# lijx10/USIP

Hardware: AMD Instinct MI355X
Metric: point-clouds/sec detector fwd+bwd (higher is better)
Workload: dtype f32 results; matrix-bound products emulated from 2 fp16 planes per operand (22-bit operands, 3 plane products, exact ...; 1 GPU; KITTI detector N=16384 M=512 K=64 batch=8 pairs/GPU (BASELINE configs[2]); detector=RPN_Detector_Ball, clouds_per_gpu=16, surface_normal_len=4, node_knn_k_1=16, ball_radius=2, ball_k=64, cloud=slab, matmul=f32x2, step=fwd+losses+bwd+adam, launch=HIP graph replay (ONE graph per step: forward, backward, Adam), parallelism=dp1

## Files before the change

include/usip_hip.h:

```cpp
#ifndef USIP_HIP_H
#define USIP_HIP_H

#include <stdint.h>

#ifdef __cplusplus
extern "C" {
#endif

#define USIP_OK      0
#define USIP_EINVAL (-1)
#define USIP_ABI 6

const char* usip_version(void);

enum { USIP_TUNE_INDEX_MAX_CH = 0, USIP_TUNE_INDEX_MAX_UNROLL, USIP_TUNE_X3_WGRAD_TILE, USIP_TUNE_X3_GEMM_TILE,
       USIP_TUNE_GEMM_SPLIT3, USIP_TUNE_INDEX_MAX_THREADS, USIP_TUNE_X2_DIRECT, USIP_TUNE_R5_FORMS, USIP_TUNE_COUNT };
int usip_set_tuning(const char* name, int value);
int usip_tuning_value(int knob);

int usip_launch_log(int on);
const char* usip_launch_log_entry(int i, unsigned* workgroups);

int usip_index_max_f32(const float* data, const int32_t* index, int32_t* max_idx,
                       int B, int C, int N, int K, void* stream);
// ... 137 lines not shown

int usip_mlp_gemm_x2d_red_tiles(int M, int K, int P, int nb, int red_group);
int usip_mlp_gemm_x2h_red_f32(const void* planes, const float* X, const float* X2, const float* coef, int pro,
                              const float* pool_dp, const int32_t* pool_arg, int pool_group, float* Y,
                              const float* red_y, const float* red_coef, float* red_out, float* red_gsum,
                              int red_group, int M, int K, int P, int nb, void* stream);
int usip_mlp_gemm_x2h_fork_supported(int M, int K, int P, int nb, int fork_group);
int usip_mlp_gemm_x2h_fork_f32(const void* planes, const float* X, const float* X2, const float* coef, float* Y, int y_rows,
                               const float* fork_dp, const int32_t* fork_arg, int fork_group, int M, int K, int P, int nb,
                               void* stream);
int usip_mlp_gemm_x2r_tiles(int P, int nb);
int usip_mlp_gemm_x2r_f32(const void* planes, const float* X, const float* X2, const float* coef, int pro,
                          const float* bias, const float* rowbias, int rb_group, const float* pool_dp,
                          const int32_t* pool_arg, int pool_group, float* Y, int y_rows, float* stats, int M, int K,
                          int P, int nb, void* stream);

int usip_multi_transpose_f32(const float* src, float* dst, const int32_t* table, int ntensors, int total_tiles,
                             void* stream);

int usip_bn_finalize_f32(const float* stats, int tiles, int C, long long count,
                         const float* gamma, const float* beta, float eps, float momentum,
                         float* running_mean, float* running_var, float* mean, float* invstd,
                         float* coef, void* stream);

int usip_bn_apply_f32(const float* Y, const float* coef, float* Z, int relu,
                      int nb, int C, int P, void* stream);

int usip_bn_backward_reduce_f32(const float* dZ, const float* Y, const float* coef_fwd,
                                const float* mean, const float* invstd, const float* gamma, int relu,
                                float* partial, float* dgamma, float* dbeta, float* coef4,
// ... 52 lines not shown
                        float* workspace, float* dW, int ldw, int coloff,
                        int M, int N, int P, int nb, void* stream);
int usip_mlp_wgrad_x2h_f32(const float* G, const float* G2, const float* coef, int pro, const float* X,
                        const float* xcoef, const float* pool_dp, const int32_t* pool_arg, int pool_group,
                        float* workspace, float* dW, int ldw, int coloff,
                        int M, int N, int P, int nb, void* stream);
int usip_mlp_wgrad_f32x3_used(int M, int N, int P, int nb);

int usip_group_gather_f32(const float* x, const int32_t* idx, const float* sub, float* out,
                          int B, int C, int N, int M, int K, int nsub, int Ctot, int coff, void* stream);
int usip_group_gather_backward_f32(const float* dout, const int32_t* idx, float* dx,
                                   int B, int C, int N, int M, int K, int Ctot, int coff, void* stream);
int usip_group_max_f32(const float* z, float* pooled, int32_t* arg, long long rows, int K, void* stream);
int usip_group_max_act_f32(const float* y, const float* coef, int relu, float* pooled, int32_t* arg, float* yarg,
                           int B, int C, int M, int K, void* stream);
int usip_group_max_backward_f32(const float* dpooled, const int32_t* arg, float* dz,
                                long long rows, int K, void* stream);
int usip_group_max_backward_add_f32(const float* dpooled, const int32_t* arg, float* dz,
                                    long long rows, int K, void* stream);

int usip_group_max_wide_f32(const float* y, const float* coef, int relu, float* pooled, int32_t* arg, float* yarg,
                            int B, int C, int M, int K, void* stream);
int usip_bn_backward_reduce_wide_f32(const float* dZ, const float* Y, const float* coef_fwd,
                                     const float* mean, const float* invstd, const float* gamma, int relu,
                                     float* partial, float* dgamma, float* dbeta, float* coef4,
                                     float* gsum, int group, int nb, int C, int P, int want_bound, void* stream);

int usip_knn_f32(const float* query, const float* database, int32_t* idx,
                 int B, int M, int N, int K, void* stream);

// ... 367 lines not shown
```

usip_amd/csrc/group.hip:

```cpp
#include "common.h"
#include "pool_order.h"

namespace {

__global__ __launch_bounds__(256) void group_gather_kernel(
    const float* __restrict__ x, const int32_t* __restrict__ idx, const float* __restrict__ sub,
    float* __restrict__ out, int C, int N, int M, int K, int nsub, int Ctot, int coff)
{
    const int b = blockIdx.y;
    const int P = M * K;
    const int p = blockIdx.x * 256 + threadIdx.x;
    if (p >= P) return;
    const int n = idx[(long long)b * P + p];
    const int m = p / K;
    const float* xb = x + (long long)b * C * N;
    float* ob = out + ((long long)b * Ctot + coff) * P;
    for (int c = 0; c < C; ++c) {
        float v = xb[(long long)c * N + n];
        if (c < nsub) v -= sub[((long long)b * nsub + c) * M + m];
        ob[(long long)c * P + p] = v;
    }
}

__global__ __launch_bounds__(256) void group_gather_bwd_kernel(
// ... 45 lines not shown
{
    return __builtin_bit_cast(float, __builtin_amdgcn_update_dpp(0, __builtin_bit_cast(int, v), CTRL, 0xF, 0xF, false));
}
template <int CTRL>
__device__ __forceinline__ int dpp_i(int v) { return __builtin_amdgcn_update_dpp(0, v, CTRL, 0xF, 0xF, false); }

template <int L, int CTRL>
__device__ __forceinline__ void argmax_step(float& best, int& bk, float& braw)
{
    const float ov = dpp_f<CTRL>(best);
    const int ok = dpp_i<CTRL>(bk);
    const float orw = dpp_f<CTRL>(braw);
    if (ov > best || (ov == best && ok < bk)) { best = ov; bk = ok; braw = orw; }
}

template <int L, bool NANS>
__global__ __launch_bounds__(256) void group_max4_kernel(
    const float* __restrict__ z, float* __restrict__ pooled, int32_t* __restrict__ arg, long long rows,
    const float* __restrict__ coef, int relu, int C, int M, float* __restrict__ zarg, int nbatch)
{
    constexpr int RPB = 256 / L, RPT = 4;
    const int sub = threadIdx.x % L;
    const bool small = rows < (1LL << 31);
    const long long first = (long long)blockIdx.x * nbatch;
    auto row_of = [&](long long batch, int j) { return batch * RPB * RPT + threadIdx.x / L + (long long)j * RPB; };
    float4 v[RPT], nv[RPT];
#pragma unroll
    for (int j = 0; j < RPT; ++j) v[j] = usip_load_stream4(z + (min(row_of(first, j), rows - 1) * L + sub) * 4);
    for (int bi = 0; bi < nbatch; ++bi) {
        const long long batch = first + bi;
        if (bi + 1 < nbatch) {
#pragma unroll
            for (int j = 0; j < RPT; ++j) nv[j] = usip_load_stream4(z + (min(row_of(batch + 1, j), rows - 1) * L + sub) * 4);
        }
#pragma unroll
        for (int j = 0; j < RPT; ++j) {
            const long long row = row_of(batch, j);
            float4 w = v[j];
            if (coef) {
                const int ch = small ? (int)(((unsigned)min(row, rows - 1) / (unsigned)M) % (unsigned)C)
                                     : (int)((min(row, rows - 1) / M) % C);
                const float s0 = coef[ch], s1 = coef[C + ch];
                w.x = __builtin_fmaf(w.x, s0, s1); w.y = __builtin_fmaf(w.y, s0, s1);
                w.z = __builtin_fmaf(w.z, s0, s1); w.w = __builtin_fmaf(w.w, s0, s1);
                if (relu) { w.x = fmaxf(w.x, 0.f); w.y = fmaxf(w.y, 0.f); w.z = fmaxf(w.z, 0.f); w.w = fmaxf(w.w, 0.f); }
            }
            float best = w.x, braw = v[j].x;
            int bk = sub * 4;
            if (pool_gt<NANS>(w.y, best)) { best = w.y; bk = sub * 4 + 1; braw = v[j].y; }
            if (pool_gt<NANS>(w.z, best)) { best = w.z; bk = sub * 4 + 2; braw = v[j].z; }
            if (pool_gt<NANS>(w.w, best)) { best = w.w; bk = sub * 4 + 3; braw = v[j].w; }
            if constexpr (NANS) pool_hide_nan(best, bk);
            if constexpr (L == 4 || L == 16) {
                argmax_step<L, 0xB1>(best, bk, braw);
                argmax_step<L, 0x4E>(best, bk, braw);
                if constexpr (L == 16) {
                    argmax_step<L, 0x141>(best, bk, braw);
                    argmax_step<L, 0x140>(best, bk, braw);
                }
            } else {
#pragma unroll
                for (int off = L / 2; off > 0; off >>= 1) {
                    const float ov = __shfl_xor(best, off);
                    const int ok = __shfl_xor(bk, off);
                    const float orw = __shfl_xor(braw, off);
                    if (ov > best || (ov == best && ok < bk)) { best = ov; bk = ok; braw = orw; }
                }
            }
            if (sub == 0 && row < rows) {
                if constexpr (NANS) {
                    if (bk < 0) { bk += POOL_NAN; best = coef ? __builtin_nanf("") : braw; }
                }
                pooled[row] = best;
                arg[row] = bk;
                if (zarg) zarg[row] = braw;
            }
        }
#pragma unroll
        for (int j = 0; j < RPT; ++j) v[j] = nv[j];
    }
}

static int group_max4_batches(long long batches)
{
    if (!(usip_tuning_value(USIP_TUNE_R5_FORMS) & 8)) return 1;
    int nb = 1;
    while (nb < 8 && batches / (nb * 2) >= 2048) nb *= 2;
    return nb;
}

__global__ __launch_bounds__(256) void group_max_bwd4_kernel(
    const float* __restrict__ dpooled, const int32_t* __restrict__ arg, float* __restrict__ dz,
    long long total4, int K4)
{
    const long long i = (long long)blockIdx.x * 256 + threadIdx.x;
    if (i >= total4) return;
    const long long row = i / K4;
    const int k = (int)(i - row * K4) * 4;
    const int a = arg[row] - k;
    const float g = dpooled[row];
    *reinterpret_cast<float4*>(dz + i * 4) =
        make_float4(a == 0 ? g : 0.f, a == 1 ? g : 0.f, a == 2 ? g : 0.f, a == 3 ? g : 0.f);
}
// ... 135 lines not shown
        const long long blocks = (batches + nbatch - 1) / nbatch;                                \
        if (blocks > 0x7fffffffLL) return USIP_EINVAL;                                           \
        if (relu)                                                                                \
            USIP_LAUNCH((group_max4_kernel<L_, false>), dim3((unsigned)blocks), dim3(256), 0, st, y, pooled, arg, rows, \
                        coef, relu, C, M, yarg, nbatch);                                        \
        else                                                                                     \
            USIP_LAUNCH((group_max4_kernel<L_, true>), dim3((unsigned)blocks), dim3(256), 0, st, y, pooled, arg, rows, \
                        coef, relu, C, M, yarg, nbatch);                                        \
    }
    USIP_GM4(1) USIP_GM4(2) USIP_GM4(4) USIP_GM4(8) USIP_GM4(16) USIP_GM4(32) USIP_GM4(64)
#undef USIP_GM4
    USIP_LAUNCH_CHECK();
    return USIP_OK;
}

extern "C" int usip_group_max_f32(const float* z, float* pooled, int32_t* arg, long long rows, int K,
                                  void* stream)
{
    if (rows < 0 || K < 1) return USIP_EINVAL;
    if (rows == 0) return USIP_OK;
    if (!z || !pooled || !arg) return USIP_EINVAL;
    hipStream_t st = (hipStream_t)stream;
    const int L4 = K / 4;
    if (K % 4 == 0 && (L4 & (L4 - 1)) == 0 && L4 <= 64 && (reinterpret_cast<uintptr_t>(z) & 15u) == 0) {
#define USIP_GM4(L_)                                                                             \
        if (L4 == L_) {                                                                          \
            const long long batches = (rows + 4 * (256 / L_) - 1) / (4 * (256 / L_));            \
            const int nbatch = group_max4_batches(batches);                                      \
            const long long blocks = (batches + nbatch - 1) / nbatch;                            \
            if (blocks > 0x7fffffffLL) return USIP_EINVAL;                                       \
// ... 59 lines not shown
```

usip_amd/csrc/shared_mlp_x3.hip:

```cpp
#include "mlp_common.h"
#include "split_common.h"
#include <type_traits>

using namespace usip_mlp;

namespace {

constexpr int X2H_PARTS = 32;

__device__ __forceinline__ float* x2h_trailer(const usip_split3_desc& d)
{
    const int bm = d.tile_rows, ksteps = (d.K + XBK - 1) / XBK;
    return reinterpret_cast<float*>(reinterpret_cast<unsigned char*>(d.planes) +
                                    (long long)((d.M + bm - 1) / bm) * ksteps * 2 * bm * 32);
}

__device__ __forceinline__ void absmax_part(const usip_split3_desc& d, int part)
{
    __shared__ float red[4];
    const long long total = (long long)d.M * d.K, per = (total + X2H_PARTS - 1) / X2H_PARTS;
    const long long i0 = part * per, i1 = i0 + per < total ? i0 + per : total;
    float mx = 0.f;
    for (long long i = i0 + threadIdx.x; i < i1; i += 256) {
        const int k = (int)(i / d.M), m = (int)(i % d.M);
// ... 744 lines not shown
#undef USIP_X2L_PRODUCT
#undef USIP_X2L_READ_FRAGS
    {
        const float out_scale = 1.0f / (gscale * xscale);
#pragma unroll
        for (int i = 0; i < TM; ++i)
#pragma unroll
            for (int j = 0; j < TN; ++j)
#pragma unroll
                for (int r = 0; r < 16; ++r) acc[i][j][r] *= out_scale;
    }
    wgrad_store_partial<TM, TN>(a, acc, slice, m0, n0, wm, wn, lane);
}


template <int PRO, int EPI, bool RB = false>
__global__ __launch_bounds__(256) __attribute__((amdgpu_waves_per_eu(2, 2))) void gemm_x2r_kernel(const GemmArgs a, const uint4* __restrict__ planes)
{
    constexpr bool POOL = (PRO == PRO_BN_BWD_POOL);
    constexpr bool TWO = (PRO == PRO_BN_BWD) || POOL;
    constexpr int NCOEF = TWO ? 4 : 2;
    constexpr int BN = 64, SLAB = 64, PLB = BN * SLAB * 2;
    __shared__ __attribute__((aligned(16))) unsigned char Bs[2][2][PLB];
    __shared__ float cf[NCOEF][128];
    __shared__ float redm[4];
    __shared__ float rbs[RB ? 2 : 1][RB ? 128 : 1][2];

    const int tid = threadIdx.x, lane = tid & 63;
    const int wave = __builtin_amdgcn_readfirstlane(tid >> 6);
    const int c = lane & 31, kh = lane >> 5;
    const int nk = (a.K + XBK - 1) / XBK;
    const int nslab = (a.K + SLAB - 1) / SLAB;
// ... 24 lines not shown
    bf16x8 fa[8][2];
    {
        const int row = wave * 32 + c;
        const int chunk = row * 2 + ((kh ^ (row >> 3)) & 1);
#pragma unroll
        for (int s8 = 0; s8 < 8; ++s8)
#pragma unroll
            for (int pl = 0; pl < 2; ++pl) {
                uint4 v = make_uint4(0u, 0u, 0u, 0u);
                if (s8 < nk) v = planes[(long long)(s8 * 2 + pl) * 256 + chunk];
                fa[s8][pl] = __builtin_bit_cast(bf16x8, v);
            }
    }
    __shared__ float bsh[128];
    if (tid < 128) bsh[tid] = (a.bias && tid < a.M) ? a.bias[tid] : 0.f;
    float s1[EPI == EPI_STATS ? 16 : 1], s2[EPI == EPI_STATS ? 16 : 1];
    if (EPI == EPI_STATS) {
#pragma unroll
        for (int r = 0; r < 16; ++r) { s1[r] = 0.f; s2[r] = 0.f; }
    }

    const int xp = tid & 63;
    const int xkg = wave;
    const int pgrp = POOL ? a.P / a.pool_group : 0;
    const unsigned cloud_bytes = (unsigned)a.K * (unsigned)a.P * 4u, pool_bytes = (unsigned)a.K * (unsigned)pgrp * 4u;

    struct Raw { float x[16]; float y[TWO ? 16 : 1]; int arg[POOL ? 16 : 1]; int xkin; float rb; };
    const int ngrp = RB ? a.P / a.rb_group : 0;
    auto load_slab = [&](int tile, int sl, Raw& r) {
        const int b = tile / tpc, p0 = (tile - b * tpc) * BN;
// ... 95 lines not shown
                        acc[j] = __builtin_amdgcn_mfma_f32_32x32x16_f16(__builtin_bit_cast(f16x8, w0), __builtin_bit_cast(f16x8, fb[1][j]), acc[j], 0, 0, 0);
                        acc[j] = __builtin_amdgcn_mfma_f32_32x32x16_f16(__builtin_bit_cast(f16x8, w1), __builtin_bit_cast(f16x8, fb[0][j]), acc[j], 0, 0, 0);
                        acc[j] = __builtin_amdgcn_mfma_f32_32x32x16_f16(__builtin_bit_cast(f16x8, w0), __builtin_bit_cast(f16x8, fb[0][j]), acc[j], 0, 0, 0);
                    }
                }
            }
        }
        if (q + 1 < nsteps) {
            store_slab(cur ^ 1, slab_of(q + 1), nxt, ((q + 1) / nslab) & 1);
            if (q + 1 + DIST < nsteps) load_slab(tile_of(q + 1 + DIST), slab_of(q + 1 + DIST), nxt);
        }
        if (sl == nslab - 1) {
            const int tile = tile_of(q);
            const int b = tile / tpc, pt = tile - b * tpc, p0 = pt * BN;
            float* yb = a.Y + (long long)b * a.y_rows * a.P;
#pragma unroll
            for (int j = 0; j < 2; ++j) {
                const int pp = p0 + j * 32 + c;
                const bool pok = pp < a.P;
#pragma unroll
                for (int r = 0; r < 16; ++r) {
                    const int ch = wave * 32 + 8 * (r >> 2) + 4 * kh + (r & 3);
                    float v = __builtin_fmaf(acc[j][r], out_scale, bsh[ch]);
                    if (RB) v += rbs[RB ? (q / nslab) & 1 : 0][RB ? ch : 0][j];
                    if (pok && ch < a.M) {
                        st_out<RB ? ST_X2R : ST_X2R_PLAIN>(yb + (long long)ch * a.P + pp, v);
                        if (EPI == EPI_STATS) { s1[EPI == EPI_STATS ? r : 0] += v; s2[EPI == EPI_STATS ? r : 0] = __builtin_fmaf(v, v, s2[EPI == EPI_STATS ? r : 0]); }
                    }
                }
            }
#pragma unroll
            for (int j = 0; j < 2; ++j)
#pragma unroll
                for (int r = 0; r < 16; ++r) acc[j][r] = 0.f;
        }
        asm volatile("s_waitcnt lgkmcnt(0)" ::: "memory");
        __builtin_amdgcn_s_barrier();
        cur ^= 1;
    };
    for (int q = 0; q < nsteps; q += 2) {
        step(q, DIST == 2 ? rB : rA);
        if (q + 1 < nsteps) step(q + 1, rA);
    }
    if (EPI == EPI_STATS) {
#pragma unroll
        for (int r = 0; r < 16; ++r) {
            float u = usip_row16_sum(s1[EPI == EPI_STATS ? r : 0]), v = usip_row16_sum(s2[EPI == EPI_STATS ? r : 0]);
            u += __shfl_xor(u, 16);
            v += __shfl_xor(v, 16);
            const int ch = wave * 32 + 8 * (r >> 2) + 4 * kh + (r & 3);
            if (c == 0 && ch < a.M) {
                a.stats[(long long)ch * G + blockIdx.x] = u;
                a.stats[(long long)G * a.M + (long long)ch * G + blockIdx.x] = v;
            }
        }
    }
}

}

extern "C" int usip_mlp_x3p_tile_rows(int M, int P, int nb)
{
    const int t = usip_tuning_value(USIP_TUNE_X3_GEMM_TILE);
    if (M <= 128 || t == 1) return 128;
    const long long wide = (long long)((M + 255) / 256) * nb * ((P + 127) / 128);
    return wide >= 256 ? 256 : 128;
}


extern "C" long long usip_mlp_split3_bytes(int M, int K)
{
// ... 215 lines not shown
    if (pro == PRO_AFFINE_RELU && rowbias) {
        if (stats) USIP_LAUNCH((gemm_x2r_kernel<PRO_AFFINE_RELU, EPI_STATS, true>), dim3(grid), dim3(256), 0, st, a, pl);
        else USIP_LAUNCH((gemm_x2r_kernel<PRO_AFFINE_RELU, EPI_NONE, true>), dim3(grid), dim3(256), 0, st, a, pl);
    } else if (pro == PRO_AFFINE_RELU) {
        if (stats) USIP_LAUNCH((gemm_x2r_kernel<PRO_AFFINE_RELU, EPI_STATS>), dim3(grid), dim3(256), 0, st, a, pl);
        else USIP_LAUNCH((gemm_x2r_kernel<PRO_AFFINE_RELU, EPI_NONE>), dim3(grid), dim3(256), 0, st, a, pl);
    } else if (pro == PRO_BN_BWD) {
        USIP_LAUNCH((gemm_x2r_kernel<PRO_BN_BWD, EPI_NONE>), dim3(grid), dim3(256), 0, st, a, pl);
    } else {
        USIP_LAUNCH((gemm_x2r_kernel<PRO_BN_BWD_POOL, EPI_NONE>), dim3(grid), dim3(256), 0, st, a, pl);
    }
    USIP_LAUNCH_CHECK();
    return USIP_OK;
}

namespace usip_mlp {

void wgrad_x3_plan(int M, int N, int P, int nb, int* seglen, int* segs, int* tiles)
{
    *tiles = ((M + 255) / 256) * ((N + 255) / 256);
    long long want = (usip_tuning_value(USIP_TUNE_X3_WGRAD_TILE) == 2 ? 512 : 256) / (*tiles);
    if (want < 1) want = 1;
    long long per_cloud = (want + nb - 1) / nb;
    if (per_cloud < 1) per_cloud = 1;
    long long sl = (P + per_cloud - 1) / per_cloud;
    sl = ((sl + 31) / 32) * 32;
    long long floor_sl = 512;
    if (usip_tuning_value(USIP_TUNE_X3_WGRAD_TILE) != 4)
        while (floor_sl > 128 && (long long)(*tiles) * nb * ((P + floor_sl - 1) / floor_sl) < 192) floor_sl /= 2;
    if (sl < floor_sl) sl = floor_sl;
// ... 36 lines not shown
```

usip_amd/functional.py:

```python
from typing import Optional, Tuple

import torch
import torch.nn.functional as F

from . import ops, prof


GRAD_SINK = False
DEFER_BN_COUNTERS = False


FUSED_NARROW_BWD = True
FUSED_NARROW_RED = True
import os as _os
if _os.environ.get("USIP_NARROW_BWD") is not None:
    FUSED_NARROW_BWD = _os.environ["USIP_NARROW_BWD"] not in ("0", "off")
if _os.environ.get("USIP_NARROW_RED") is not None:
    FUSED_NARROW_RED = _os.environ["USIP_NARROW_RED"] not in ("0", "off")


SEGMENT_BACKWARD = _os.environ.get("USIP_SEGMENT_BWD", "1") not in ("0", "off")


WT_CACHE = None
# ... 502 lines not shown
                dw = ops.mlp_wgrad(dz, x, pro=2, G2=y, coef4=coef4, xcoef=xcoef,
                                   out=sink[0].view(w2.shape) if sink else None)
        db = torch.zeros_like(gamma) if (ctx.needs_input_grad[3] and not sink) else None
        if sink:
            dw = db = dgamma = dbeta = None
        return (dx, None, dw, db, dgamma, dbeta) + tail


class _SharedMLPLayerMax(torch.autograd.Function):

    @staticmethod
    def forward(ctx, x, xcoef, dims, w2, bias, gamma, beta, running_mean, running_var, momentum, eps, sink):
        B, Cin, M, K = dims
        x3 = x.contiguous().view(B, Cin, M * K)
        Cout = w2.shape[0]
        y, stats = ops.mlp_gemm(_kmajor(w2), x3, bias, want_stats=True,
                                pro=0 if xcoef is None else 1, coef=xcoef)
        mean, invstd, coef = ops.bn_finalize(stats, B * M * K, gamma, beta, eps, momentum, running_mean, running_var)
        y = _relu_hook(y, coef)
        pooled, arg, yarg = _pooled_act(y.view(B, Cout, M, K), coef, True, want_yarg=True)
        ctx.save_for_backward(x3, xcoef, w2, y, coef, mean, invstd, gamma, arg, yarg)
        ctx.dims, ctx.sink, ctx.x_shape = (B, Cin, Cout, M, K), sink, tuple(x.shape)
        return pooled

    @staticmethod
    def backward(ctx, dpooled):
        x3, xcoef, w2, y, coef, mean, invstd, gamma, arg, yarg = ctx.saved_tensors
        B, Cin, Cout, M, K = ctx.dims
        sink = ctx.sink
        dpooled = dpooled.contiguous()
        dgamma, dbeta, coef4 = ops.bn_pool_backward_reduce(dpooled, arg, y.view(B, Cout, M, K), coef, mean, invstd,
                                                           gamma, True, dgamma_out=sink[2] if sink else None,
                                                           dbeta_out=sink[3] if sink else None, yarg=yarg)
        pool = (dpooled, arg, K)
        dx = dw = None
# ... 536 lines not shown
```

usip_amd/ops.py:

```python
import ctypes
import functools
import math
import os
import types
from typing import Callable, NamedTuple, Optional

import torch

from . import _lib, prof


def _stream(t: torch.Tensor):
    return ctypes.c_void_p(torch.cuda.current_stream(t.device).cuda_stream)


def _need(t: torch.Tensor, name: str, dtype):
    if not isinstance(t, torch.Tensor):
        raise RuntimeError("%s must be a torch.Tensor" % name)
    if not t.is_cuda:
        raise RuntimeError("%s must be a CUDA tensor/variable" % name)
    if not t.is_contiguous():
        raise RuntimeError("%s must be contiguous" % name)
    if t.dtype != dtype:
        raise RuntimeError("%s must be %s (got %s)" % (name, dtype, t.dtype))
# ... 489 lines not shown
        dt = np.dtype(_lib.STRUCTS["usip_split3_desc"])
        table = np.array(rows, dtype=dt) if rows else np.zeros(0, dtype=dt)
        dev = next(iter(self.entries.values()))[1].device if rows else None
        self.table = torch.from_numpy(table.view(np.uint8).copy()).to(dev) if rows else None

    def refresh(self):
        if self.table is not None:
            with torch.cuda.device(self.table.device), prof.kernel("weight_split3", 0.0):
                _lib.check(_lib.lib().usip_mlp_split3_multi_f32(_ptr(self.table), len(self.entries), self.blocks,
                                                                _stream(self.table)), "usip_mlp_split3_multi_f32")
        return dict(self.entries)


NARROW_FWD = _os.environ.get("USIP_NARROW_FWD", "1") not in ("0", "off")
POOL_GRAD_FOLD = _os.environ.get("USIP_POOL_GRAD_FOLD", "1") not in ("0", "off")


def mlp_gemm(At: torch.Tensor, X: torch.Tensor, bias=None, want_stats: bool = False, pro: int = 0,
             X2=None, coef=None, tag: str = "fwd", rowbias=None, rb_group: int = 1,
             M: Optional[int] = None, a_offset: int = 0, pool=None, a_trans: bool = False, out=None,
             out_row_offset: int = 0, red=None, red_group: int = 0, fork=None):
    _need(At, "At", torch.float32)
    if a_trans:
        M_rows, lda = At.shape
        M = M_rows if M is None else int(M)
        K = X2.shape[1] if X is None else X.shape[1]
    else:
        K, lda = At.shape
        M = lda if M is None else int(M)
    pool_dp = pool_arg = None
    pool_group = 0
    if pool is not None:
        pool_dp, pool_arg, pool_group = pool
        X = X2
    _need(X, "X", torch.float32)
    nb, Kx, P = X.shape
# ... 47 lines not shown
    red_tiles = 0
    if (red is not None and plain_dgrad and out is None
            and red[1] is not None and red[1].shape[0] >= 4 and tuple(red[0].shape) == (nb, M, P)
            and red[0].is_contiguous() and red[0].data_ptr() % 16 == 0):
        red_tiles = int(lib.usip_mlp_gemm_x2d_red_tiles(M, K, P, nb, int(red_group)))
    fork_fold = False
    if fork is not None and plain_dgrad and pro == 2 and red is None and not want_stats and POOL_GRAD_FOLD:
        f_dp, f_arg, f_group = fork
        _need(f_dp, "fork dpooled", torch.float32)
        _need(f_arg, "fork arg", torch.int32)
        fork_fold = bool(f_group > 0 and P % f_group == 0 and tuple(f_dp.shape) == (nb, M, P // f_group)
                         and f_arg.shape == f_dp.shape and f_dp.data_ptr() % 16 == 0 and f_arg.data_ptr() % 16 == 0
                         and X.data_ptr() % 16 == 0 and X2.data_ptr() % 16 == 0 and y_ptr.value % 16 == 0
                         and lib.usip_mlp_gemm_x2h_fork_supported(M, K, P, nb, int(f_group)))
    third = None
    x_ptr = None if pool is not None else _ptr(X)
    epi = (_opt(coef), int(pro), _opt(bias), _opt(rowbias), int(rb_group))
    pooled = (_opt(pool_dp), _opt(pool_arg), int(pool_group))
    shape = (M, K, P, nb, _stream(X))
    if nf_blocks:
        fn, args = "usip_mlp_narrow_forward_f32", (a_ptr, lda, x_ptr) + epi + (y_ptr, int(y_rows), _opt(stats))
    elif red_tiles:
        flat = torch.empty(2 * red_tiles * M + red_tiles * (M // 256), dtype=torch.float32, device=X.device)
        third = RedSums(flat, M, blocks=red_tiles)
        third.gsum = torch.empty((2, nb, M, P // red_group), dtype=torch.float32, device=X.device) if red_group else None
        fn, args = "usip_mlp_gemm_x2h_red_f32", (_ptr(planes), x_ptr, _opt(X2), _opt(coef), int(pro)) + pooled + (
            y_ptr, _ptr(red[0]), _ptr(red[1]), _ptr(flat), _opt(third.gsum), int(red_group))
    elif fork_fold:
        third = True
        fn, args = "usip_mlp_gemm_x2h_fork_f32", (_ptr(planes), _ptr(X), _ptr(X2), _ptr(coef), y_ptr, int(y_rows),
                                                  _ptr(f_dp), _ptr(f_arg), int(f_group))
    else:
        fn = (("usip_mlp_gemm_x2r_f32" if x2r else "usip_mlp_gemm_x2h_f32" if x2h else "usip_mlp_gemm_x3p_f32") if x3p else
              {"bf16": "usip_mlp_gemm_bf16", "f32x3": "usip_mlp_gemm_f32x3", "f32x2": "usip_mlp_gemm_f32x3"}.get(
                  _matmul_mode, "usip_mlp_gemm_f32"))
        args = ((_ptr(planes),) if x3p else (a_ptr, -lda if a_trans else lda)) + (x_ptr, _opt(X2)) + epi + pooled + (
            y_ptr, int(y_rows), _opt(stats))
    with torch.cuda.device(X.device), prof.kernel("shared_mlp_gemm_%s %dx%d" % (tag, M, K),
                                                  4.0 * nb * P * (K * (2 if pro == 2 else 1) + M),
                                                  2.0 * M * K * nb * P, keyed=True, moved=moved):
        _lib.check(getattr(lib, fn)(*args, *shape), fn)
    return (Y, stats, third) if red is not None else ((Y, stats, bool(third)) if fork is not None else (Y, stats))


def bn_finalize(stats, count, gamma, beta, eps, momentum, running_mean, running_var):
    _, C, tiles = stats.shape
    dev = stats.device
    mean = torch.empty(C, dtype=torch.float32, device=dev)
    invstd = torch.empty(C, dtype=torch.float32, device=dev)
    coef = torch.empty((4, C), dtype=torch.float32, device=dev)
    with torch.cuda.device(dev), prof.kernel("bn_finalize", 4.0 * 2 * tiles * C):
        _lib.check(_lib.lib().usip_bn_finalize_f32(_ptr(stats), tiles, C, int(count), _opt(gamma), _opt(beta),
                                                   float(eps), float(momentum), _opt(running_mean),
                                                   _opt(running_var), _ptr(mean), _ptr(invstd), _ptr(coef),
                                                   _stream(stats)), "usip_bn_finalize_f32")
    declare_samples(coef, int(count))
# ... 398 lines not shown
    return pooled, arg


def group_max_act(y4, coef, relu: bool, want_yarg: bool = False):
    _need(y4, "y", torch.float32)
    B, C, M, K = y4.shape
    pooled = torch.empty((B, C, M), dtype=torch.float32, device=y4.device)
    arg = torch.empty((B, C, M), dtype=torch.int32, device=y4.device)
    yarg = torch.empty((B, C, M), dtype=torch.float32, device=y4.device) if want_yarg else None
    with torch.cuda.device(y4.device), prof.kernel("group_max", 4.0 * B * C * M * (K + 2)):
        _lib.check(_lib.lib().usip_group_max_act_f32(_ptr(y4), _ptr(coef), int(bool(relu)), _ptr(pooled), _ptr(arg),
                                                     _opt(yarg), B, C, M, K, _stream(y4)), "usip_group_max_act_f32")
    return (pooled, arg, yarg) if want_yarg else (pooled, arg)


WIDE_GROUPS = os.environ.get("USIP_WIDE_GROUPS", "1") not in ("0", "off")


def wide_group_supported(K: int) -> bool:
    return bool(WIDE_GROUPS) and 256 < K <= 1024 and K % 32 == 0


def group_max_wide(y4, coef=None, relu: bool = False, want_yarg: bool = False):
    _need(y4, "y", torch.float32)
    B, C, M, K = y4.shape
    pooled = torch.empty((B, C, M), dtype=torch.float32, device=y4.device)
    arg = torch.empty((B, C, M), dtype=torch.int32, device=y4.device)
    yarg = torch.empty((B, C, M), dtype=torch.float32, device=y4.device) if want_yarg else None
    with torch.cuda.device(y4.device), prof.kernel("group_max_wide", 4.0 * B * C * M * (K + 2)):
        _lib.check(_lib.lib().usip_group_max_wide_f32(_ptr(y4), _opt(coef), int(bool(relu)), _ptr(pooled), _ptr(arg),
# ... 1706 lines not shown
```

Measured before the change: 4109 point-clouds/s.

## Fuse max-pool candidate scan into GEMM epilogue with cheap resolve kernel

The x2r GEMM epilogue now scans each 64-wide K group per output channel and records the top pre-activation value, the runner-up, the first element and the argmax, using the sign of gamma as the order key. A small resolve kernel then applies the BN affine and ReLU to those records to produce pooled, arg and yarg. It falls back to a full row rescan only on ties, non-finite values or sign mismatches. This is meant to avoid re-reading the whole Y tensor in a separate group-max pass, at the cost of extra LDS traffic and registers in the GEMM epilogue and a small candidate buffer.

After: 4136 point-clouds/s, median of 6. Within noise of the previous version (+0.7%).

```diff
diff --git a/include/usip_hip.h b/include/usip_hip.h
--- a/include/usip_hip.h
+++ b/include/usip_hip.h
@@ -175,6 +175,9 @@
                           const float* bias, const float* rowbias, int rb_group, const float* pool_dp,
                           const int32_t* pool_arg, int pool_group, float* Y, int y_rows, float* stats, int M, int K,
                           int P, int nb, void* stream);
+int usip_mlp_gemm_x2r_cand_f32(const void* planes, const float* X, const float* coef, const float* bias,
+                               const float* gamma, float* Y, int y_rows, float* stats, void* cand, int M, int K, int P,
+                               int nb, void* stream);
 
 int usip_multi_transpose_f32(const float* src, float* dst, const int32_t* table, int ntensors, int total_tiles,
                              void* stream);
@@ -257,6 +260,9 @@
 int usip_group_max_f32(const float* z, float* pooled, int32_t* arg, long long rows, int K, void* stream);
 int usip_group_max_act_f32(const float* y, const float* coef, int relu, float* pooled, int32_t* arg, float* yarg,
                            int B, int C, int M, int K, void* stream);
+int usip_pool_resolve_f32(const void* cand, const float* y, const float* coef, const float* gamma, int relu,
+                          float* pooled, int32_t* arg, float* yarg, int B, int C, int M, void* nfallback,
+                          void* stream);
 int usip_group_max_backward_f32(const float* dpooled, const int32_t* arg, float* dz,
                                 long long rows, int K, void* stream);
 int usip_group_max_backward_add_f32(const float* dpooled, const int32_t* arg, float* dz,
diff --git a/usip_amd/csrc/group.hip b/usip_amd/csrc/group.hip
--- a/usip_amd/csrc/group.hip
+++ b/usip_amd/csrc/group.hip
@@ -1,5 +1,6 @@
 #include "common.h"
 #include "pool_order.h"
+#include "pool_cand.h"
 
 namespace {
 
@@ -83,6 +84,48 @@
     if (ov > best || (ov == best && ok < bk)) { best = ov; bk = ok; braw = orw; }
 }
 
+__device__ __forceinline__ float4 pool_act4(float4 w, float s0, float s1, int relu)
+{
+    w.x = __builtin_fmaf(w.x, s0, s1); w.y = __builtin_fmaf(w.y, s0, s1);
+    w.z = __builtin_fmaf(w.z, s0, s1); w.w = __builtin_fmaf(w.w, s0, s1);
+    if (relu) { w.x = fmaxf(w.x, 0.f); w.y = fmaxf(w.y, 0.f); w.z = fmaxf(w.z, 0.f); w.w = fmaxf(w.w, 0.f); }
+    return w;
+}
+
+template <int L, bool NANS>
+__device__ __forceinline__ void pool_row4(const float4 raw, const float4 w, int sub, float& best, int& bk, float& braw)
+{
+    best = w.x; braw = raw.x;
+    bk = sub * 4;
+    if (pool_gt<NANS>(w.y, best)) { best = w.y; bk = sub * 4 + 1; braw = raw.y; }
+    if (pool_gt<NANS>(w.z, best)) { best = w.z; bk = sub * 4 + 2; braw = raw.z; }
+    if (pool_gt<NANS>(w.w, best)) { best = w.w; bk = sub * 4 + 3; braw = raw.w; }
+    if constexpr (NANS) pool_hide_nan(best, bk);
+    if constexpr (L == 4 || L == 16) {
+        argmax_step<L, 0xB1>(best, bk, braw);
+        argmax_step<L, 0x4E>(best, bk, braw);
+        if constexpr (L == 16) {
+            argmax_step<L, 0x141>(best, bk, braw);
+            argmax_step<L, 0x140>(best, bk, braw);
+        }
+    } else {
+#pragma unroll
+        for (int off = L / 2; off > 0; off >>= 1) {
+            const float ov = __shfl_xor(best, off);
+            const int ok = __shfl_xor(bk, off);
+            const float orw = __shfl_xor(braw, off);
+            if (ov > best || (ov == best && ok < bk)) { best = ov; bk = ok; braw = orw; }
+        }
+    }
+}
+template <bool NANS>
+__device__ __forceinline__ void pool_row4_unhide(bool acted, float& best, int& bk, float braw)
+{
+    if constexpr (NANS) {
+        if (bk < 0) { bk += POOL_NAN; best = acted ? __builtin_nanf("") : braw; }
+    }
+}
+
 template <int L, bool NANS>
 __global__ __launch_bounds__(256) void group_max4_kernel(
     const float* __restrict__ z, float* __restrict__ pooled, int32_t* __restrict__ arg, long long rows,
@@ -109,37 +152,13 @@
             if (coef) {
                 const int ch = small ? (int)(((unsigned)min(row, rows - 1) / (unsigned)M) % (unsigned)C)
                                      : (int)((min(row, rows - 1) / M) % C);
-                const float s0 = coef[ch], s1 = coef[C + ch];
-                w.x = __builtin_fmaf(w.x, s0, s1); w.y = __builtin_fmaf(w.y, s0, s1);
-                w.z = __builtin_fmaf(w.z, s0, s1); w.w = __builtin_fmaf(w.w, s0, s1);
-                if (relu) { w.x = fmaxf(w.x, 0.f); w.y = fmaxf(w.y, 0.f); w.z = fmaxf(w.z, 0.f); w.w = fmaxf(w.w, 0.f); }
+                w = pool_act4(w, coef[ch], coef[C + ch], relu);
             }
-            float best = w.x, braw = v[j].x;
-            int bk = sub * 4;
-            if (pool_gt<NANS>(w.y, best)) { best = w.y; bk = sub * 4 + 1; braw = v[j].y; }
-            if (pool_gt<NANS>(w.z, best)) { best = w.z; bk = sub * 4 + 2; braw = v[j].z; }
-            if (pool_gt<NANS>(w.w, best)) { best = w.w; bk = sub * 4 + 3; braw = v[j].w; }
-            if constexpr (NANS) pool_hide_nan(best, bk);
-            if constexpr (L == 4 || L == 16) {
-                argmax_step<L, 0xB1>(best, bk, braw);
-                argmax_step<L, 0x4E>(best, bk, braw);
-                if constexpr (L == 16) {
-                    argmax_step<L, 0x141>(best, bk, braw);
-                    argmax_step<L, 0x140>(best, bk, braw);
-                }
-            } else {
-#pragma unroll
-                for (int off = L / 2; off > 0; off >>= 1) {
-                    const float ov = __shfl_xor(best, off);
-                    const int ok = __shfl_xor(bk, off);
-                    const float orw = __shfl_xor(braw, off);
-                    if (ov > best || (ov == best && ok < bk)) { best = ov; bk = ok; braw = orw; }
-                }
-            }
+            float best, braw;
+            int bk;
+            pool_row4<L, NANS>(v[j], w, sub, best, bk, braw);
             if (sub == 0 && row < rows) {
-                if constexpr (NANS) {
-                    if (bk < 0) { bk += POOL_NAN; best = coef ? __builtin_nanf("") : braw; }
-                }
+                pool_row4_unhide<NANS>(coef != nullptr, best, bk, braw);
                 pooled[row] = best;
                 arg[row] = bk;
                 if (zarg) zarg[row] = braw;
@@ -156,6 +175,51 @@
     int nb = 1;
     while (nb < 8 && batches / (nb * 2) >= 2048) nb *= 2;
     return nb;
+}
+
+template <bool RELU>
+__global__ __launch_bounds__(256) void pool_resolve_kernel(
+    const float4* __restrict__ cand, const float* __restrict__ y, const float* __restrict__ coef,
+    const float* __restrict__ gamma, float* __restrict__ pooled, int32_t* __restrict__ arg, float* __restrict__ yarg,
+    int rows, int C, int M, unsigned* __restrict__ nfallback)
+{
+    const int lane = threadIdx.x & 63;
+    const int row = blockIdx.x * 256 + threadIdx.x, rowc = min(row, rows - 1);
+    const int ch = (int)(((unsigned)rowc / (unsigned)M) % (unsigned)C);
+    const float sc = coef[ch], sh = coef[C + ch];
+    const float4 rec = cand[rowc];
+    const int ktop = __float_as_int(rec.w);
+    auto act = [&](float t) { const float w = __builtin_fmaf(t, sc, sh); return RELU ? fmaxf(w, 0.f) : w; };
+    const float v = act(rec.x);
+    const bool neg = (__float_as_uint(gamma[ch]) >> 31) != 0, scneg = (__float_as_uint(sc) >> 31) != 0;
+    bool fb = ktop < 0 || !(fabsf(sc) < __builtin_inff()) || !(fabsf(sh) < __builtin_inff()) || (sc != 0.f && neg != scneg);
+    float p = v, ya = rec.x;
+    int a = ktop;
+    if (!fb) {
+        if (RELU && v == 0.f) { p = act(rec.z); a = 0; ya = rec.z; }
+        else if (act(rec.y) == v) fb = true;
+    }
+    unsigned long long todo = __ballot(fb && row < rows);
+    if (nfallback && todo && lane == 0) atomicAdd(nfallback, (unsigned)__popcll(todo));
+    while (todo) {
+        const int src = __ffsll((long long)todo) - 1;
+        todo &= todo - 1;
+        const int frow = __shfl(rowc, src);
+        const float fsc = __shfl(sc, src), fsh = __shfl(sh, src);
+        const int sub = lane & 15;
+        const float4 raw = *reinterpret_cast<const float4*>(y + ((long long)frow * 16 + sub) * 4);
+        const float4 w = pool_act4(raw, fsc, fsh, RELU ? 1 : 0);
+        float best, braw;
+        int bk;
+        pool_row4<16, !RELU>(raw, w, sub, best, bk, braw);
+        pool_row4_unhide<!RELU>(true, best, bk, braw);
+        if (lane == src) { p = best; a = bk; ya = braw; }
+    }
+    if (row < rows) {
+        pooled[row] = p;
+        arg[row] = a;
+        if (yarg) yarg[row] = ya;
+    }
 }
 
 __global__ __launch_bounds__(256) void group_max_bwd4_kernel(
@@ -321,6 +385,26 @@
     return USIP_OK;
 }
 
+extern "C" int usip_pool_resolve_f32(const void* cand, const float* y, const float* coef, const float* gamma, int relu,
+                                     float* pooled, int32_t* arg, float* yarg, int B, int C, int M, void* nfallback,
+                                     void* stream)
+{
+    const long long rows = (long long)B * C * M;
+    if (B < 0 || C < 1 || M < 0 || rows >= (1LL << 31) - 256) return USIP_EINVAL;
+    if (rows == 0) return USIP_OK;
+    if (!cand || !y || !coef || !gamma || !pooled || !arg) return USIP_EINVAL;
+    if ((reinterpret_cast<uintptr_t>(y) | reinterpret_cast<uintptr_t>(cand)) & 15u) return USIP_EINVAL;
+    hipStream_t st = (hipStream_t)stream;
+    const dim3 grid((unsigned)((rows + 255) / 256));
+    const float4* rec = reinterpret_cast<const float4*>(cand);
+    if (relu)
+        USIP_LAUNCH((pool_resolve_kernel<true>), grid, dim3(256), 0, st, rec, y, coef, gamma, pooled, arg, yarg, (int)rows, C, M, reinterpret_cast<unsigned*>(nfallback));
+    else
+        USIP_LAUNCH((pool_resolve_kernel<false>), grid, dim3(256), 0, st, rec, y, coef, gamma, pooled, arg, yarg, (int)rows, C, M, reinterpret_cast<unsigned*>(nfallback));
+    USIP_LAUNCH_CHECK();
+    return USIP_OK;
+}
+
 extern "C" int usip_group_max_f32(const float* z, float* pooled, int32_t* arg, long long rows, int K,
                                   void* stream)
 {
diff --git a/usip_amd/csrc/pool_cand.h b/usip_amd/csrc/pool_cand.h
--- /dev/null
+++ b/usip_amd/csrc/pool_cand.h
@@ -0,0 +1,54 @@
+#pragma once
+#include "common.h"
+
+struct PoolCandScan {
+    float top, next;
+    int k;
+    unsigned amax;
+};
+
+__device__ __forceinline__ float pool_cand_key(float y, unsigned smask)
+{
+    return __uint_as_float(__float_as_uint(y) ^ smask);
+}
+
+__device__ __forceinline__ void pool_cand_first(PoolCandScan& s, float y, unsigned smask, int k0)
+{
+    s.top = pool_cand_key(y, smask);
+    s.next = -__builtin_inff();
+    s.k = k0;
+    s.amax = __float_as_uint(y) & 0x7fffffffu;
+}
+
+__device__ __forceinline__ void pool_cand_push(PoolCandScan& s, float y, unsigned smask, int k)
+{
+    const float t = pool_cand_key(y, smask);
+    const bool gt = t > s.top, lt = t < s.top;
+    const float lo = gt ? s.top : t;
+    s.next = ((gt || lt) && lo > s.next) ? lo : s.next;
+    s.k = gt ? k : s.k;
+    s.top = gt ? t : s.top;
+    const unsigned ab = __float_as_uint(y) & 0x7fffffffu;
+    s.amax = ab > s.amax ? ab : s.amax;
+}
+
+template <int CTRL>
+__device__ __forceinline__ void pool_cand_merge(PoolCandScan& s)
+{
+    const float ot = __builtin_bit_cast(float, __builtin_amdgcn_update_dpp(0, __builtin_bit_cast(int, s.top), CTRL, 0xF, 0xF, false));
+    const float on = __builtin_bit_cast(float, __builtin_amdgcn_update_dpp(0, __builtin_bit_cast(int, s.next), CTRL, 0xF, 0xF, false));
+    const int ok = __builtin_amdgcn_update_dpp(0, s.k, CTRL, 0xF, 0xF, false);
+    const unsigned oa = (unsigned)__builtin_amdgcn_update_dpp(0, (int)s.amax, CTRL, 0xF, 0xF, false);
+    const bool eq = ot == s.top, win = ot > s.top || (eq && ok < s.k);
+    const float c0 = eq ? s.next : (win ? s.top : ot), c1 = (eq || win) ? on : s.next;
+    s.next = c0 > c1 ? c0 : c1;
+    s.top = win ? ot : s.top;
+    s.k = win ? ok : s.k;
+    s.amax = oa > s.amax ? oa : s.amax;
+}
+
+__device__ __forceinline__ float4 pool_cand_record(const PoolCandScan& s, unsigned smask, float y0)
+{
+    const int k = s.amax >= 0x7f800000u ? -1 : s.k;
+    return make_float4(pool_cand_key(s.top, smask), pool_cand_key(s.next, smask), y0, __int_as_float(k));
+}
diff --git a/usip_amd/csrc/shared_mlp_x3.hip b/usip_amd/csrc/shared_mlp_x3.hip
--- a/usip_amd/csrc/shared_mlp_x3.hip
+++ b/usip_amd/csrc/shared_mlp_x3.hip
@@ -1,5 +1,6 @@
 #include "mlp_common.h"
 #include "split_common.h"
+#include "pool_cand.h"
 #include <type_traits>
 
 using namespace usip_mlp;
@@ -782,8 +783,9 @@
 }
 
 
-template <int PRO, int EPI, bool RB = false>
-__global__ __launch_bounds__(256) __attribute__((amdgpu_waves_per_eu(2, 2))) void gemm_x2r_kernel(const GemmArgs a, const uint4* __restrict__ planes)
+template <int PRO, int EPI, bool RB, bool CAND>
+__device__ __forceinline__ void gemm_x2r_body(const GemmArgs& a, const uint4* __restrict__ planes, float4* __restrict__ cand,
+                                              const float* __restrict__ gamma)
 {
     constexpr bool POOL = (PRO == PRO_BN_BWD_POOL);
     constexpr bool TWO = (PRO == PRO_BN_BWD) || POOL;
@@ -838,6 +840,14 @@
     }
     __shared__ float bsh[128];
     if (tid < 128) bsh[tid] = (a.bias && tid < a.M) ? a.bias[tid] : 0.f;
+    unsigned smask[2] = {0u, 0u};
+    if constexpr (CAND) {
+#pragma unroll
+        for (int h = 0; h < 2; ++h) {
+            const int ch = wave * 32 + 16 * h + (lane >> 2);
+            if (ch < a.M) smask[h] = __float_as_uint(gamma[ch]) & 0x80000000u;
+        }
+    }
     float s1[EPI == EPI_STATS ? 16 : 1], s2[EPI == EPI_STATS ? 16 : 1];
     if (EPI == EPI_STATS) {
 #pragma unroll
@@ -963,19 +973,49 @@
             const int tile = tile_of(q);
             const int b = tile / tpc, pt = tile - b * tpc, p0 = pt * BN;
             float* yb = a.Y + (long long)b * a.y_rows * a.P;
-#pragma unroll
-            for (int j = 0; j < 2; ++j) {
-                const int pp = p0 + j * 32 + c;
-                const bool pok = pp < a.P;
-#pragma unroll
-                for (int r = 0; r < 16; ++r) {
-                    const int ch = wave * 32 + 8 * (r >> 2) + 4 * kh + (r & 3);
-                    float v = __builtin_fmaf(acc[j][r], out_scale, bsh[ch]);
-                    if (RB) v += rbs[RB ? (q / nslab) & 1 : 0][RB ? ch : 0][j];
-                    if (pok && ch < a.M) {
-                        st_out<RB ? ST_X2R : ST_X2R_PLAIN>(yb + (long long)ch * a.P + pp, v);
-                        if (EPI == EPI_STATS) { s1[EPI == EPI_STATS ? r : 0] += v; s2[EPI == EPI_STATS ? r : 0] = __builtin_fmaf(v, v, s2[EPI == EPI_STATS ? r : 0]); }
+            constexpr int NH = CAND ? 2 : 1, RH = 16 / NH;
+            constexpr int CROW = 68;
+            __shared__ __attribute__((aligned(16))) float cimg[CAND ? 4 : 1][CAND ? 16 * CROW : 4];
+#pragma unroll
+            for (int h = 0; h < NH; ++h) {
+#pragma unroll
+                for (int j = 0; j < 2; ++j) {
+                    const int pp = p0 + j * 32 + c;
+                    const bool pok = pp < a.P;
+#pragma unroll
+                    for (int rr = 0; rr < RH; ++rr) {
+                        const int r = h * RH + rr;
+                        const int ch = wave * 32 + 8 * (r >> 2) + 4 * kh + (r & 3);
+                        float v = __builtin_fmaf(acc[j][r], out_scale, bsh[ch]);
+                        if (RB) v += rbs[RB ? (q / nslab) & 1 : 0][RB ? ch : 0][j];
+                        if (pok && ch < a.M) {
+                            st_out<RB ? ST_X2R : ST_X2R_PLAIN>(yb + (long long)ch * a.P + pp, v);
+                            if (EPI == EPI_STATS) { s1[EPI == EPI_STATS ? r : 0] += v; s2[EPI == EPI_STATS ? r : 0] = __builtin_fmaf(v, v, s2[EPI == EPI_STATS ? r : 0]); }
+                        }
+                        if constexpr (CAND) cimg[wave][(8 * (rr >> 2) + 4 * kh + (rr & 3)) * CROW + j * 32 + c] = v;
                     }
+                }
+                if constexpr (CAND) {
+                    const float* img = cimg[wave];
+                    const int chl = lane >> 2, run = lane & 3;
+                    asm volatile("s_waitcnt lgkmcnt(0)" ::: "memory");
+                    PoolCandScan ps;
+                    float y0 = 0.f;
+#pragma unroll
+                    for (int i = 0; i < 4; ++i) {
+                        const float4 q4 = *reinterpret_cast<const float4*>(&img[chl * CROW + run * 16 + i * 4]);
+                        if (i == 0) { pool_cand_first(ps, q4.x, smask[h], run * 16); y0 = q4.x; }
+                        else pool_cand_push(ps, q4.x, smask[h], run * 16 + i * 4);
+                        pool_cand_push(ps, q4.y, smask[h], run * 16 + i * 4 + 1);
+                        pool_cand_push(ps, q4.z, smask[h], run * 16 + i * 4 + 2);
+                        pool_cand_push(ps, q4.w, smask[h], run * 16 + i * 4 + 3);
+                    }
+                    asm volatile("s_waitcnt lgkmcnt(0)" ::: "memory");
+                    pool_cand_merge<0xB1>(ps);
+                    pool_cand_merge<0x4E>(ps);
+                    const int ch = wave * 32 + 16 * h + chl;
+                    if (run == 0 && ch < a.M)
+                        cand[((long long)b * a.M + ch) * tpc + pt] = pool_cand_record(ps, smask[h], y0);
                 }
             }
 #pragma unroll
@@ -1004,6 +1044,19 @@
             }
         }
     }
+}
+
+template <int PRO, int EPI, bool RB = false>
+__global__ __launch_bounds__(256) __attribute__((amdgpu_waves_per_eu(2, 2))) void gemm_x2r_kernel(const GemmArgs a, const uint4* __restrict__ planes)
+{
+    gemm_x2r_body<PRO, EPI, RB, false>(a, planes, nullptr, nullptr);
+}
+
+template <int EPI>
+__global__ __launch_bounds__(256) __attribute__((amdgpu_waves_per_eu(2, 2))) void gemm_x2r_cand_kernel(
+    const GemmArgs a, const uint4* __restrict__ planes, float4* __restrict__ cand, const float* __restrict__ gamma)
+{
+    gemm_x2r_body<PRO_AFFINE_RELU, EPI, false, true>(a, planes, cand, gamma);
 }
 
 }
@@ -1249,6 +1302,28 @@
     return USIP_OK;
 }
 
+extern "C" int usip_mlp_gemm_x2r_cand_f32(const void* planes, const float* X, const float* coef, const float* bias,
+                                          const float* gamma, float* Y, int y_rows, float* stats, void* cand, int M,
+                                          int K, int P, int nb, void* stream)
+{
+    if (M < 1 || M > 128 || K < 1 || K > 128 || P < 64 || P % 64 != 0 || nb < 1) return USIP_EINVAL;
+    if ((long long)K * P >= (1LL << 30)) return USIP_EINVAL;
+    if (!planes || !gamma || !cand || ((reinterpret_cast<uintptr_t>(planes) | reinterpret_cast<uintptr_t>(cand)) & 15u))
+        return USIP_EINVAL;
+    GemmArgs a;
+    if (!gemm_entry_args(a, X, nullptr, coef, PRO_AFFINE_RELU, bias, nullptr, 1, nullptr, nullptr, 0, Y, y_rows, stats,
+                         M, K, P, nb)) return USIP_EINVAL;
+    a.rb_group = 1;
+    const long long total = (long long)nb * (P / 64);
+    const unsigned grid = (unsigned)(total < 512 ? total : 512);
+    hipStream_t st = (hipStream_t)stream;
+    const uint4* pl = reinterpret_cast<const uint4*>(planes);
+    if (stats) USIP_LAUNCH((gemm_x2r_cand_kernel<EPI_STATS>), dim3(grid), dim3(256), 0, st, a, pl, reinterpret_cast<float4*>(cand), gamma);
+    else USIP_LAUNCH((gemm_x2r_cand_kernel<EPI_NONE>), dim3(grid), dim3(256), 0, st, a, pl, reinterpret_cast<float4*>(cand), gamma);
+    USIP_LAUNCH_CHECK();
+    return USIP_OK;
+}
+
 namespace usip_mlp {
 
 void wgrad_x3_plan(int M, int N, int P, int nb, int* seglen, int* segs, int* tiles)
diff --git a/usip_amd/functional.py b/usip_amd/functional.py
--- a/usip_amd/functional.py
+++ b/usip_amd/functional.py
@@ -540,11 +540,19 @@
         B, Cin, M, K = dims
         x3 = x.contiguous().view(B, Cin, M * K)
         Cout = w2.shape[0]
-        y, stats = ops.mlp_gemm(_kmajor(w2), x3, bias, want_stats=True,
-                                pro=0 if xcoef is None else 1, coef=xcoef)
+        in_producer = ops.POOL_IN_PRODUCER and K == 64 and xcoef is not None and not pins_active()
+        cand = None
+        if in_producer:
+            y, stats, cand = ops.mlp_gemm(_kmajor(w2), x3, bias, want_stats=True, pro=1, coef=xcoef, cand_gamma=gamma)
+        else:
+            y, stats = ops.mlp_gemm(_kmajor(w2), x3, bias, want_stats=True,
+                                    pro=0 if xcoef is None else 1, coef=xcoef)
         mean, invstd, coef = ops.bn_finalize(stats, B * M * K, gamma, beta, eps, momentum, running_mean, running_var)
         y = _relu_hook(y, coef)
-        pooled, arg, yarg = _pooled_act(y.view(B, Cout, M, K), coef, True, want_yarg=True)
+        if cand is not None:
+            pooled, arg, yarg = ops.pool_resolve(cand, y.view(B, Cout, M, K), coef, gamma, True, want_yarg=True)
+        else:
+            pooled, arg, yarg = _pooled_act(y.view(B, Cout, M, K), coef, True, want_yarg=True)
         ctx.save_for_backward(x3, xcoef, w2, y, coef, mean, invstd, gamma, arg, yarg)
         ctx.dims, ctx.sink, ctx.x_shape = (B, Cin, Cout, M, K), sink, tuple(x.shape)
         return pooled
diff --git a/usip_amd/ops.py b/usip_amd/ops.py
--- a/usip_amd/ops.py
+++ b/usip_amd/ops.py
@@ -527,12 +527,13 @@
 
 NARROW_FWD = _os.environ.get("USIP_NARROW_FWD", "1") not in ("0", "off")
 POOL_GRAD_FOLD = _os.environ.get("USIP_POOL_GRAD_FOLD", "1") not in ("0", "off")
+POOL_IN_PRODUCER = _os.environ.get("USIP_POOL_IN_PRODUCER", "1") not in ("0", "off")
 
 
 def mlp_gemm(At: torch.Tensor, X: torch.Tensor, bias=None, want_stats: bool = False, pro: int = 0,
              X2=None, coef=None, tag: str = "fwd", rowbias=None, rb_group: int = 1,
              M: Optional[int] = None, a_offset: int = 0, pool=None, a_trans: bool = False, out=None,
-             out_row_offset: int = 0, red=None, red_group: int = 0, fork=None):
+             out_row_offset: int = 0, red=None, red_group: int = 0, fork=None, cand_gamma=None):
     _need(At, "At", torch.float32)
     if a_trans:
         M_rows, lda = At.shape
@@ -610,11 +611,19 @@
                          and X.data_ptr() % 16 == 0 and X2.data_ptr() % 16 == 0 and y_ptr.value % 16 == 0
                          and lib.usip_mlp_gemm_x2h_fork_supported(M, K, P, nb, int(f_group)))
     third = None
+    cand = None
+    if (cand_gamma is not None and x2r and pro == 1 and want_stats and rowbias is None and out is None and P % 64 == 0
+            and red is None and fork is None and pool is None and X2 is None and tuple(cand_gamma.shape) == (M,)
+            and cand_gamma.dtype == torch.float32 and cand_gamma.is_contiguous() and cand_gamma.device == X.device):
+        cand = torch.empty((nb, M, P // 64, 4), dtype=torch.float32, device=X.device)
     x_ptr = None if pool is not None else _ptr(X)
     epi = (_opt(coef), int(pro), _opt(bias), _opt(rowbias), int(rb_group))
     pooled = (_opt(pool_dp), _opt(pool_arg), int(pool_group))
     shape = (M, K, P, nb, _stream(X))
-    if nf_blocks:
+    if cand is not None:
+        fn, args = "usip_mlp_gemm_x2r_cand_f32", (_ptr(planes), x_ptr, _ptr(coef), _opt(bias), _ptr(cand_gamma), y_ptr,
+                                                  int(y_rows), _ptr(stats), _ptr(cand))
+    elif nf_blocks:
         fn, args = "usip_mlp_narrow_forward_f32", (a_ptr, lda, x_ptr) + epi + (y_ptr, int(y_rows), _opt(stats))
     elif red_tiles:
         flat = torch.empty(2 * red_tiles * M + red_tiles * (M // 256), dtype=torch.float32, device=X.device)
@@ -636,6 +645,8 @@
                                                   4.0 * nb * P * (K * (2 if pro == 2 else 1) + M),
                                                   2.0 * M * K * nb * P, keyed=True, moved=moved):
         _lib.check(getattr(lib, fn)(*args, *shape), fn)
+    if cand_gamma is not None:
+        return Y, stats, cand
     return (Y, stats, third) if red is not None else ((Y, stats, bool(third)) if fork is not None else (Y, stats))
 
 
@@ -1064,6 +1075,22 @@
     return (pooled, arg, yarg) if want_yarg else (pooled, arg)
 
 
+def pool_resolve(cand, y4, coef, gamma, relu: bool, want_yarg: bool = False, count=None):
+    _need(y4, "y", torch.float32)
+    _need(cand, "cand", torch.float32)
+    B, C, M, K = y4.shape
+    if K != 64 or tuple(cand.shape) != (B, C, M, 4):
+        raise RuntimeError("pool_resolve: records %s do not belong to a pool over %s" % (tuple(cand.shape), tuple(y4.shape)))
+    pooled = torch.empty((B, C, M), dtype=torch.float32, device=y4.device)
+    arg = torch.empty((B, C, M), dtype=torch.int32, device=y4.device)
+    yarg = torch.empty((B, C, M), dtype=torch.float32, device=y4.device) if want_yarg else None
+    with torch.cuda.device(y4.device), prof.kernel("pool_resolve", 4.0 * B * C * M * (4 + 3)):
+        _lib.check(_lib.lib().usip_pool_resolve_f32(_ptr(cand), _ptr(y4), _ptr(coef), _ptr(gamma), int(bool(relu)),
+                                                    _ptr(pooled), _ptr(arg), _opt(yarg), B, C, M, _opt(count),
+                                                    _stream(y4)), "usip_pool_resolve_f32")
+    return (pooled, arg, yarg) if want_yarg else (pooled, arg)
+
+
 WIDE_GROUPS = os.environ.get("USIP_WIDE_GROUPS", "1") not in ("0", "off")
 
 
```
